# soasme/LTX-Video-GPUPoor

Hardware: AMD Instinct MI355X
Metric: denoise-steps/sec + VAE-decode frames/sec, LTX-Video 768x512x97f at 1/8 GPU (higher is better)
Workload: dtype bf16

## Files before the change

### include/ltxmi.h

```cpp
#ifndef LTXMI_H
#define LTXMI_H

#include <stddef.h>
#include <stdint.h>

#ifdef __cplusplus
extern "C" {
#endif

typedef enum ltxmi_status {
    LTXMI_OK = 0,
    LTXMI_ERR_INVALID_ARG = -1,
    LTXMI_ERR_UNSUPPORTED = -2,
    LTXMI_ERR_LAUNCH = -3
} ltxmi_status;

const char* ltxmi_version(void);
const char* ltxmi_last_error(void);
const char* ltxmi_arch(void);

typedef enum ltxmi_epilogue {
    LTXMI_EPI_NONE = 0,
    LTXMI_EPI_GELU_TANH = 1,
    LTXMI_EPI_SILU = 2,
// ... 37 lines not shown
                             const void* scale_table, const void* scale_temb,
                             const void* shift_table, const void* shift_temb,
                             int64_t temb_ld, int32_t rows_per_group, void* stream);

int ltxmi_norm_modulate_f32in_bf16(const float* x, int64_t ldx, void* y, int64_t ldy,
                                   int32_t rows, int32_t D, float eps, int32_t kind,
                                   const void* scale_table, const void* scale_temb,
                                   const void* shift_table, const void* shift_temb,
                                   int64_t temb_ld, int32_t rows_per_group, void* stream);

int ltxmi_gate_residual_f32(float* h, int64_t ldh, const void* y, int64_t ldy, int32_t rows, int32_t D,
                            const void* gate_table, const void* gate_temb, int64_t gate_ld,
                            int32_t rows_per_group, int32_t round_product,
                            void* h_bf16, int64_t ld_h_bf16, void* stream);

int ltxmi_rmsnorm_rope_bf16(void* x, int64_t ldx, int32_t rows, int32_t D,
                            const void* weight, float eps,
                            const void* cos_tab, const void* sin_tab, int64_t ld_tab,
                            int32_t rope_period, void* stream);
int ltxmi_rmsnorm_rope_rstd_bf16(void* x, int64_t ldx, int32_t rows, int32_t D, const void* weight, float eps,
                                 const void* cos_tab, const void* sin_tab, int64_t ld_tab, int32_t rope_period,
                                 const float* rowsumsq, int64_t rowsumsq_ld, int32_t rowsumsq_blocks,
                                 int32_t norm_dim, float norm_eps, float* rstd_out, void* stream);

typedef struct ltxmi_attn_args {
    const void* q; int64_t q_stride_b, q_stride_l;
    const void* k; int64_t k_stride_b, k_stride_l;
    const void* v; int64_t v_stride_b, v_stride_l;
    void*       o; int64_t o_stride_b, o_stride_l;
    const float* key_bias; int64_t bias_stride_b;
    int32_t B, H, Lq, Lk, head_dim;
    float   softmax_scale;
    const float* q_rowsumsq; int64_t q_rowsumsq_stride_b, q_rowsumsq_stride_l; int32_t q_rowsumsq_blocks;
    const void*  q_norm_weight; float q_norm_eps;
    const void*  rope_cos; const void* rope_sin; int64_t rope_stride_b, rope_stride_l;
    int32_t o_segment_len; int64_t o_stride_segment;
    const float* q_rstd; int64_t q_rstd_stride_b, q_rstd_stride_l;
    uint32_t* redo_counter; int32_t force_exact;
    float* lse; int64_t lse_stride_b, lse_stride_h;
} ltxmi_attn_args;

int ltxmi_attention_fwd_bf16(const ltxmi_attn_args* args, void* stream);
int ltxmi_attention_fuses_qnorm(int32_t B, int32_t H, int32_t Lq, int32_t Lk, int32_t head_dim, int32_t has_key_bias);
int ltxmi_attention_kernel_id(int32_t B, int32_t H, int32_t Lq, int32_t Lk, int32_t head_dim, int32_t has_key_bias,
                              int64_t k_stride_l, int64_t v_stride_l);

// ... 123 lines not shown
```

### ltx-video-gpupoor_amd/csrc/rowops.hip

```cpp
#include "common.h"

namespace ltxmi {

constexpr int ROWS_PER_WG = 4;

struct Chunk {
    float v[8];
};
__device__ __forceinline__ Chunk load_chunk(const uint16_t* p) {
    const u32x4 w = *(const u32x4*)p;
    Chunk c;
#pragma unroll
    for (int i = 0; i < 4; ++i) {
        c.v[2 * i] = bf_lo(w[i]);
        c.v[2 * i + 1] = bf_hi(w[i]);
    }
    return c;
}
__device__ __forceinline__ void store_chunk(uint16_t* p, const Chunk& c) {
    u32x4 w;
#pragma unroll
    for (int i = 0; i < 4; ++i) w[i] = pack_bf16(c.v[2 * i], c.v[2 * i + 1]);
    *(u32x4*)p = w;
}
// ... 88 lines not shown
    }
    s2 = wave_sum(s2);
    const float rstd = rsqrtf(s2 / D + eps);
    const int64_t trow = cs ? (int64_t)(row % rope_period) * ld_tab : 0;
#pragma unroll
    for (int j = 0; j < NCH; ++j) {
        const int ch = lane + 64 * j;
        if (ch < nchunk) {
            const Chunk wt = load_chunk(w + ch * 8);
            Chunk o;
#pragma unroll
            for (int e = 0; e < 8; ++e) o.v[e] = c[j].v[e] * rstd * wt.v[e];
            if (cs) {
                const Chunk co = load_chunk(cs + trow + ch * 8), si = load_chunk(sn + trow + ch * 8);
                Chunk r2;
#pragma unroll
                for (int e = 0; e < 8; e += 2) {
                    r2.v[e] = o.v[e] * co.v[e] - o.v[e + 1] * si.v[e];
                    r2.v[e + 1] = o.v[e + 1] * co.v[e + 1] + o.v[e] * si.v[e + 1];
                }
                o = r2;
            }
            store_chunk(xr + ch * 8, o);
        }
    }
}

template <int NCH>
__global__ __launch_bounds__(256) void pixelnorm_ada_silu_kernel(const uint16_t* __restrict__ x,
                                                                 uint16_t* __restrict__ y, int64_t rows, int C,
                                                                 int64_t rows_per_batch,
                                                                 const float* __restrict__ scale,
                                                                 const float* __restrict__ shift, int apply_silu,
                                                                 float eps) {
    const int lane = threadIdx.x & 63;
    const int64_t row = (int64_t)blockIdx.x * ROWS_PER_WG + (threadIdx.x >> 6);
    if (row >= rows) return;
    const int nchunk = C >> 3;
    const uint16_t* xr = x + row * C;
    Chunk c[NCH];
    float s2 = 0.f;
#pragma unroll
    for (int j = 0; j < NCH; ++j) {
        const int ch = lane + 64 * j;
        if (ch < nchunk) {
            c[j] = load_chunk(xr + ch * 8);
// ... 294 lines not shown
    return check_launch("ltxmi_rmsnorm_rope_bf16");
}

extern "C" int ltxmi_qkv_norm_rope_pack_bf16(const void* qkv, int64_t ld, int32_t B, int32_t Nl, int32_t D, int32_t P,
                                             const void* q_weight, const void* k_weight, float eps, const void* cos_tab,
                                             const void* sin_tab, int64_t ld_tab, int32_t rope_period, void* out,
                                             void* stream) {
    LTXMI_REQUIRE(qkv && q_weight && k_weight && out, LTXMI_ERR_INVALID_ARG, "ltxmi_qkv_norm_rope_pack_bf16: NULL argument");
    LTXMI_REQUIRE((cos_tab == nullptr) == (sin_tab == nullptr), LTXMI_ERR_INVALID_ARG,
                  "ltxmi_qkv_norm_rope_pack_bf16: cos and sin must both be given or both be NULL");
    LTXMI_REQUIRE(B > 0 && Nl > 0 && D > 0 && P > 0, LTXMI_ERR_INVALID_ARG, "ltxmi_qkv_norm_rope_pack_bf16: non-positive size");
    LTXMI_REQUIRE(D % (8 * P) == 0 && D <= 8192 && ld % 8 == 0 && ld >= 3 * D, LTXMI_ERR_UNSUPPORTED,
                  "ltxmi_qkv_norm_rope_pack_bf16: D=%d must be a multiple of 8 * P (P=%d) and <= 8192, ld >= 3 D", D, P);
    LTXMI_REQUIRE((int64_t)B * Nl < (1ll << 31) - 4, LTXMI_ERR_UNSUPPORTED, "ltxmi_qkv_norm_rope_pack_bf16: too many rows");
    if (cos_tab) LTXMI_REQUIRE(rope_period > 0 && ld_tab % 8 == 0 && ld_tab >= D, LTXMI_ERR_INVALID_ARG,
                               "ltxmi_qkv_norm_rope_pack_bf16: bad rope table geometry");
    const int rows = B * Nl, grid = (rows + ROWS_PER_WG - 1) / ROWS_PER_WG;
    hipStream_t s = (hipStream_t)stream;
    DISPATCH_NCH(D, hipLaunchKernelGGL((qkv_norm_rope_pack_kernel<NCH>), dim3(grid), dim3(256), 0, s, (const uint16_t*)qkv,
                                       ld, B, Nl, D, P, (const uint16_t*)q_weight, (const uint16_t*)k_weight, eps,
                                       (const uint16_t*)cos_tab, (const uint16_t*)sin_tab, ld_tab,
                                       rope_period > 0 ? rope_period : 1, (uint16_t*)out))
    return check_launch("ltxmi_qkv_norm_rope_pack_bf16");
}

extern "C" int ltxmi_pixelnorm_ada_silu_bf16(const void* x, void* y, int64_t rows, int32_t C,
                                             int64_t rows_per_batch, const float* scale, const float* shift,
                                             int32_t apply_silu, float eps, void* stream) {
    LTXMI_REQUIRE(x && y, LTXMI_ERR_INVALID_ARG, "ltxmi_pixelnorm_ada_silu_bf16: NULL argument");
    LTXMI_REQUIRE((scale == nullptr) == (shift == nullptr), LTXMI_ERR_INVALID_ARG,
                  "ltxmi_pixelnorm_ada_silu_bf16: scale and shift must both be given or both be NULL");
    LTXMI_REQUIRE(rows > 0 && C > 0 && rows_per_batch > 0, LTXMI_ERR_INVALID_ARG,
                  "ltxmi_pixelnorm_ada_silu_bf16: non-positive size");
    LTXMI_REQUIRE(C % 8 == 0 && C <= 8192, LTXMI_ERR_UNSUPPORTED,
                  "ltxmi_pixelnorm_ada_silu_bf16: C=%d must be a multiple of 8 and <= 8192", C);
    const int64_t grid = (rows + ROWS_PER_WG - 1) / ROWS_PER_WG;
    LTXMI_REQUIRE(grid < (1ll << 31), LTXMI_ERR_UNSUPPORTED, "ltxmi_pixelnorm_ada_silu_bf16: too many rows");
    hipStream_t s = (hipStream_t)stream;
    if ((C == 64 || C == 128 || C == 256) && ((((uintptr_t)scale | (uintptr_t)shift) & 15) == 0)) {
        const int rpw = 512 / C;
        int64_t g = (rows + ROWS_PER_WG * rpw - 1) / (ROWS_PER_WG * rpw);
        if (g > 256 * 16) g = 256 * 16;
#define CALLN(LPR_)                                                                                             \
    hipLaunchKernelGGL((pixelnorm_ada_silu_narrow_kernel<LPR_>), dim3((unsigned)g), dim3(256), 0, s,             \
                       (const uint16_t*)x, (uint16_t*)y, rows, rows_per_batch, scale, shift, apply_silu, eps)
        if (C == 64) CALLN(8);
// ... 26 lines not shown
```

### ltx-video-gpupoor_amd/ltxmi/_lib.py

```python
import ctypes
import os

import torch

_HERE = os.path.dirname(os.path.abspath(__file__))
LIB_PATH = os.environ.get("LTXMI_LIB") or os.path.join(_HERE, "libltxmi.so")

c_void_p, c_int, c_int64, c_float = ctypes.c_void_p, ctypes.c_int32, ctypes.c_int64, ctypes.c_float


class GemmArgs(ctypes.Structure):
    _fields_ = [("A", c_void_p), ("lda", c_int64), ("W", c_void_p), ("ldw", c_int64), ("bias", c_void_p),
                ("C", c_void_p), ("ldc", c_int64), ("M", c_int), ("N", c_int), ("K", c_int),
                ("epilogue", c_int), ("residual", c_void_p), ("ldr", c_int64), ("gate_table", c_void_p),
                ("gate_temb", c_void_p), ("gate_ld", c_int64), ("rows_per_group", c_int), ("algo", c_int),
                ("rowsumsq", c_void_p), ("rowsumsq_cols", c_int), ("rowsumsq_ld", c_int64),
                ("a_kblock", c_int), ("a_kblock_stride", c_int64)]


class GemmPair(ctypes.Structure):
    _fields_ = [("A2", c_void_p), ("lda2", c_int64), ("W2", c_void_p), ("ldw2", c_int64), ("K2", c_int), ("group_cols", c_int)]


class AttnArgs(ctypes.Structure):
    _fields_ = [("q", c_void_p), ("q_stride_b", c_int64), ("q_stride_l", c_int64),
                ("k", c_void_p), ("k_stride_b", c_int64), ("k_stride_l", c_int64),
                ("v", c_void_p), ("v_stride_b", c_int64), ("v_stride_l", c_int64),
                ("o", c_void_p), ("o_stride_b", c_int64), ("o_stride_l", c_int64),
                ("key_bias", c_void_p), ("bias_stride_b", c_int64),
                ("B", c_int), ("H", c_int), ("Lq", c_int), ("Lk", c_int), ("head_dim", c_int),
                ("softmax_scale", c_float),
                ("q_rowsumsq", c_void_p), ("q_rowsumsq_stride_b", c_int64), ("q_rowsumsq_stride_l", c_int64),
                ("q_rowsumsq_blocks", c_int), ("q_norm_weight", c_void_p), ("q_norm_eps", c_float),
                ("rope_cos", c_void_p), ("rope_sin", c_void_p), ("rope_stride_b", c_int64), ("rope_stride_l", c_int64),
                ("o_segment_len", c_int), ("o_stride_segment", c_int64),
                ("q_rstd", c_void_p), ("q_rstd_stride_b", c_int64), ("q_rstd_stride_l", c_int64),
                ("redo_counter", c_void_p), ("force_exact", c_int),
                ("lse", c_void_p), ("lse_stride_b", c_int64), ("lse_stride_h", c_int64)]


ATTN_MERGE_MAX = 8


class AttnMergeArgs(ctypes.Structure):
    _fields_ = [("n", c_int),
                ("o_part", c_void_p * ATTN_MERGE_MAX), ("o_part_stride_b", c_int64 * ATTN_MERGE_MAX),
                ("o_part_stride_l", c_int64 * ATTN_MERGE_MAX),
                ("lse_part", c_void_p * ATTN_MERGE_MAX), ("lse_part_stride_b", c_int64 * ATTN_MERGE_MAX),
                ("lse_part_stride_h", c_int64 * ATTN_MERGE_MAX),
                ("o", c_void_p), ("o_stride_b", c_int64), ("o_stride_l", c_int64),
                ("lse", c_void_p), ("lse_stride_b", c_int64), ("lse_stride_h", c_int64),
                ("B", c_int), ("H", c_int), ("Lq", c_int), ("head_dim", c_int)]


class Conv3dArgs(ctypes.Structure):
    _fields_ = [("x", c_void_p), ("w", c_void_p), ("bias", c_void_p), ("y", c_void_p),
                ("B", c_int), ("T", c_int), ("H", c_int), ("W", c_int), ("Cin", c_int), ("Cout", c_int),
                ("causal", c_int), ("pad_replicate", c_int), ("d2s", c_int), ("residual", c_void_p),
                ("res_channels", c_int), ("add", c_void_p),
                ("stride_t", c_int), ("stride_hw", c_int), ("tpad", c_int), ("out_T", c_int),
                ("kernel_t", c_int), ("time_pad_zeros", c_int), ("algo", c_int),
# ... 3 lines not shown

class Conv3dRouteInfo(ctypes.Structure):
    _fields_ = [("route", c_int), ("epilogue", c_int), ("ksplit", c_int), ("swap_hw", c_int), ("finalize_blocks", c_int)]


SIGNATURES = {
    "ltxmi_version": (ctypes.c_char_p, []),
    "ltxmi_last_error": (ctypes.c_char_p, []),
    "ltxmi_arch": (ctypes.c_char_p, []),
    "ltxmi_gemm_bf16": (c_int, [ctypes.POINTER(GemmArgs), c_void_p]),
    "ltxmi_gemm_kernel_id": (c_int, [ctypes.POINTER(GemmArgs)]),
    "ltxmi_gemm_pair2_bf16": (c_int, [ctypes.POINTER(GemmArgs), ctypes.POINTER(GemmPair), c_void_p]),
    "ltxmi_gemm_pair2_kernel_id": (c_int, [ctypes.POINTER(GemmArgs), ctypes.POINTER(GemmPair)]),
    "ltxmi_norm_modulate_bf16": (c_int, [c_void_p, c_int64, c_void_p, c_int64, c_int, c_int, c_float, c_int,
                                         c_void_p, c_void_p, c_void_p, c_void_p, c_int64, c_int, c_void_p]),
    "ltxmi_norm_modulate_f32in_bf16": (c_int, [c_void_p, c_int64, c_void_p, c_int64, c_int, c_int, c_float, c_int,
                                               c_void_p, c_void_p, c_void_p, c_void_p, c_int64, c_int, c_void_p]),
    "ltxmi_gate_residual_f32": (c_int, [c_void_p, c_int64, c_void_p, c_int64, c_int, c_int, c_void_p, c_void_p, c_int64,
                                        c_int, c_int, c_void_p, c_int64, c_void_p]),
    "ltxmi_rmsnorm_rope_bf16": (c_int, [c_void_p, c_int64, c_int, c_int, c_void_p, c_float, c_void_p, c_void_p,
                                        c_int64, c_int, c_void_p]),
    "ltxmi_rmsnorm_rope_rstd_bf16": (c_int, [c_void_p, c_int64, c_int, c_int, c_void_p, c_float, c_void_p, c_void_p,
                                             c_int64, c_int, c_void_p, c_int64, c_int, c_int, c_float, c_void_p, c_void_p]),
    "ltxmi_rowsumsq_rstd_f32": (c_int, [c_void_p, c_int64, c_int, c_int, c_int, c_float, c_void_p, c_void_p]),
    "ltxmi_qkv_norm_rope_pack_bf16": (c_int, [c_void_p, c_int64, c_int, c_int, c_int, c_int, c_void_p, c_void_p, c_float,
                                              c_void_p, c_void_p, c_int64, c_int, c_void_p, c_void_p]),
    "ltxmi_attention_fwd_bf16": (c_int, [ctypes.POINTER(AttnArgs), c_void_p]),
    "ltxmi_attention_merge_bf16": (c_int, [ctypes.POINTER(AttnMergeArgs), c_void_p]),
    "ltxmi_attention_fuses_qnorm": (c_int, [c_int, c_int, c_int, c_int, c_int, c_int]),
    "ltxmi_attention_kernel_id": (c_int, [c_int, c_int, c_int, c_int, c_int, c_int, c_int64, c_int64]),
    "ltxmi_silu_bf16": (c_int, [c_void_p, c_void_p, c_int64, c_void_p]),
    "ltxmi_timestep_embedding_bf16": (c_int, [c_void_p, c_void_p, c_int, c_int, c_void_p]),
    "ltxmi_stg_blend_bf16": (c_int, [c_void_p, c_int64, c_void_p, c_int64, c_void_p, c_int, c_int, c_int, c_void_p]),
    "ltxmi_stg_blend_grouped_bf16": (c_int, [c_void_p, c_void_p, c_int64, c_int64, c_int64, c_void_p, c_int, c_int, c_int, c_int,
                                             c_void_p]),
    "ltxmi_conv3d_ndhwc_bf16": (c_int, [ctypes.POINTER(Conv3dArgs), c_void_p]),
    "ltxmi_conv3d_fuses_post_norm": (c_int, [ctypes.POINTER(Conv3dArgs)]),
    "ltxmi_conv3d_workspace_bytes": (c_int64, [ctypes.POINTER(Conv3dArgs)]),
    "ltxmi_conv3d_route": (c_int, [ctypes.POINTER(Conv3dArgs), ctypes.POINTER(Conv3dRouteInfo)]),
    "ltxmi_pixelnorm_ada_silu_bf16": (c_int, [c_void_p, c_void_p, c_int64, c_int, c_int64, c_void_p, c_void_p,
                                              c_int, c_float, c_void_p]),
    "ltxmi_add_bf16": (c_int, [c_void_p, c_void_p, c_void_p, c_int64, c_void_p]),
    "ltxmi_layernorm_affine_bf16": (c_int, [c_void_p, c_void_p, c_int64, c_int, c_void_p, c_void_p, c_float,
                                            c_void_p]),
    "ltxmi_ncdhw_to_ndhwc_bf16": (c_int, [c_void_p, c_void_p, c_int, c_int, c_int, c_int, c_int, c_void_p,
                                          c_void_p, c_void_p]),
# ... 52 lines not shown
```

### ltx-video-gpupoor_amd/ltxmi/attention.py

```python
from enum import Enum, auto
from typing import Optional

import torch
from torch import nn

from . import lora, ops
from .attention_seam import pay_attention

BF16 = torch.bfloat16


FUSE_CROSS_ATTENTION_Q = True


class SkipLayerStrategy(Enum):
    AttentionSkip = auto()
    AttentionValues = auto()
    Residual = auto()
    TransformerBlock = auto()


def reshape_hidden_states(hidden_states, latent_frames):
    return hidden_states.reshape(hidden_states.shape[0], latent_frames, -1, hidden_states.shape[-1])

# ... 165 lines not shown
        else:
            wqkv, bqkv = attn.packed_qkv()
        if not isinstance(attn.q_norm, RMSNorm):
            raise NotImplementedError("ltxmi.AttnProcessor2_0: qk_norm=None is not on this path")

        q_fused = None
        if not is_cross:
            fuse_q = ops.attention_fuses_qnorm(B, H, N, N, dh) and D % 64 == 0 and attention_mask is None
            ss = torch.empty((B * N, D // 64), dtype=torch.float32, device=x2.device) if fuse_q else None
            qkv = ops.gemm(x2, wqkv, bqkv, rowsumsq=ss, rowsumsq_cols=D if fuse_q else 0,
                           **lora.pair(attn, "qkv", x2))
            q2, k2, v2 = qkv[:, :D], qkv[:, D:2 * D], qkv[:, 2 * D:]
            cos = sin = None
            period = 0
            if attn.use_rope:
                cos, sin = freqs_cis
                if cos.shape[0] not in (1, B):
                    raise ValueError("freqs_cis batch must be 1 or the batch size")
                cos2, sin2 = cos.reshape(-1, D), sin.reshape(-1, D)
                period = cos2.shape[0]
                cos, sin = cos2, sin2
            if fuse_q:
                rstd = torch.empty((B * N,), dtype=torch.float32, device=x2.device)
                ops.rmsnorm_rope_(k2, attn.k_norm.weight, attn.k_norm.eps, cos, sin, period,
                                  rstd_of=(ss, D, attn.q_norm.eps, rstd))
                q_fused = ((rstd, attn.q_norm.weight, attn.q_norm.eps), (cos, sin, period) if cos is not None else None)
            else:
                ops.rmsnorm_rope_(q2, attn.q_norm.weight, attn.q_norm.eps, cos, sin, period)
                ops.rmsnorm_rope_(k2, attn.k_norm.weight, attn.k_norm.eps, cos, sin, period)
            Lk = N
            q4 = qkv.view(B, N, 3, H, dh)[:, :, 0]
            k4 = qkv.view(B, N, 3, H, dh)[:, :, 1]
            v4 = qkv.view(B, N, 3, H, dh)[:, :, 2]
            v3 = qkv.view(B, N, 3 * D)[:, :, 2 * D:]
        else:
            Bk, Lk, _ = encoder_hidden_states.shape
            fuse_q = FUSE_CROSS_ATTENTION_Q and D % 64 == 0 and bool(ops.attention_fuses_qnorm(B, H, N, Lk, dh, attention_mask is not None))
            ss = torch.empty((B * N, D // 64), dtype=torch.float32, device=x2.device) if fuse_q else None
            q2 = ops.gemm(x2, attn.to_q.weight, attn.to_q.bias, rowsumsq=ss, rowsumsq_cols=D if fuse_q else 0,
                          **lora.pair(attn, "q", x2))
            ehs = encoder_hidden_states
            key = (ehs.data_ptr(), tuple(ehs.shape), ops.tensor_version(ehs), wkv.data_ptr(), ops.tensor_version(wkv),
                   attn.k_norm.weight.data_ptr(), ops.tensor_version(attn.k_norm.weight), lora.epoch(attn))
            cache = attn.__dict__.setdefault("_text_kv_cache", {})
            hit = cache.get(key) if ops.STEP_INVARIANT_CACHING else None
            if hit is None:
                ready = attn.__dict__.get("_text_kv_ready")
                if ready is not None:
# ... 205 lines not shown
```

### ltx-video-gpupoor_amd/ltxmi/ops.py

```python
import ctypes
import math

import torch

from . import _lib
from ._lib import lib, check

BF16 = torch.bfloat16

EPI_NONE, EPI_GELU_TANH, EPI_SILU, EPI_GATE_RESIDUAL = 0, 1, 2, 3
NORM_RMS, NORM_LAYER = 0, 1


def _stream():
    return ctypes.c_void_p(torch.cuda.current_stream().cuda_stream)


_watch = None
_events = {}


def watch_launches(keys):
    global _watch
    _watch = set(keys) if keys else None
# ... 200 lines not shown
    _chk_f32(h, "gate_residual_f32_")
    _chk_bf16(y, gate_table, gate_temb, h_bf16)
    h2, rows, ldh = _rows(h)
    y2, yrows, ldy = _rows(y)
    D = h2.shape[1]
    if yrows != rows or y2.shape[1] != D:
        raise ValueError("ltxmi.gate_residual_f32_: y must have h's rows and channels")
    if (gate_table is None) != (gate_temb is None):
        raise ValueError("ltxmi.gate_residual_f32_: gate_table and gate_temb go together")
    gate_ld = 0
    if gate_temb is not None:
        gate_ld = gate_temb.stride(0) if gate_temb.dim() == 2 else 0
    b2, ldb = None, 0
    if h_bf16 is not None:
        b2, brows, ldb = _rows(h_bf16)
        if brows != rows or b2.shape[1] != D:
            raise ValueError("ltxmi.gate_residual_f32_: h_bf16 must have h's rows and channels")
    check(lib.ltxmi_gate_residual_f32(_ptr(h2), ldh, _ptr(y2), ldy, rows, D, _ptr(gate_table), _ptr(gate_temb), gate_ld,
                                      rows_per_group, int(round_product), _ptr(b2), ldb, _stream()),
          "ltxmi_gate_residual_f32")
    return h


def rmsnorm_rope_(x, weight, eps, cos=None, sin=None, rope_period=0, rstd_of=None):
    _chk_bf16(x, weight, cos, sin)
    x2, rows, ldx = _rows(x)
    D = x2.shape[1]
    ld_tab = 0
    if cos is not None:
        if cos.dim() != 2 or cos.shape != sin.shape or cos.stride(0) != sin.stride(0):
            raise ValueError("ltxmi.rmsnorm_rope_: cos/sin must be matching 2-D tables")
        ld_tab = cos.stride(0)
        rope_period = rope_period or cos.shape[0]
    if rstd_of is not None:
        ss, norm_dim, norm_eps, out = rstd_of
        if ss.dtype != torch.float32 or out.dtype != torch.float32 or ss.dim() != 2 or ss.shape[0] != rows or \
                ss.stride(1) != 1 or out.shape != (rows,) or not out.is_contiguous():
            raise ValueError("ltxmi.rmsnorm_rope_: rstd_of needs fp32 sums [rows, blocks] and a contiguous fp32 out [rows]")
        check(lib.ltxmi_rmsnorm_rope_rstd_bf16(_ptr(x2), ldx, rows, D, _ptr(weight), eps, _ptr(cos), _ptr(sin), ld_tab,
                                               rope_period, _ptr(ss), ss.stride(0), ss.shape[1], norm_dim, norm_eps,
                                               _ptr(out), _stream()), "ltxmi_rmsnorm_rope_rstd_bf16")
        return x
    check(lib.ltxmi_rmsnorm_rope_bf16(_ptr(x2), ldx, rows, D, _ptr(weight), eps, _ptr(cos), _ptr(sin), ld_tab,
                                      rope_period, _stream()), "ltxmi_rmsnorm_rope_bf16")
    return x


def rowsumsq_rstd(ss, norm_dim, eps, out=None):
    if ss.dtype != torch.float32 or ss.dim() != 2 or ss.stride(1) != 1 or not ss.is_cuda:
        raise ValueError("ltxmi.rowsumsq_rstd: expected CUDA fp32 sums [rows, blocks]")
    rows = ss.shape[0]
    out = torch.empty((rows,), dtype=torch.float32, device=ss.device) if out is None else out
    check(lib.ltxmi_rowsumsq_rstd_f32(_ptr(ss), ss.stride(0), ss.shape[1], rows, norm_dim, eps, _ptr(out), _stream()),
          "ltxmi_rowsumsq_rstd_f32")
    return out


def attention_fuses_qnorm(B, H, Lq, Lk, dh, has_key_bias=False):
    return bool(lib.ltxmi_attention_fuses_qnorm(B, H, Lq, Lk, dh, int(has_key_bias)))


# ... 543 lines not shown
```

### ltx-video-gpupoor_amd/ltxmi/transformer3d.py

```python
import contextlib
import math
from dataclasses import dataclass
from typing import Any, Dict, List, Optional

import torch
from torch import nn

from . import lora, ops
from .attention import BasicTransformerBlock, SkipLayerStrategy

BF16 = torch.bfloat16


@dataclass
class Transformer3DModelOutput:
    sample: torch.Tensor


class _TimestepEmbedder(nn.Module):
    def __init__(self, in_channels, dim):
        super().__init__()
        self.linear_1 = nn.Linear(in_channels, dim)
        self.linear_2 = nn.Linear(dim, dim)

# ... 196 lines not shown
            sin_freq = torch.cat([torch.zeros_like(cos_freq[:, :, : dim % 6]), sin_freq], dim=-1)
        return cos_freq.to(self.dtype).contiguous(), sin_freq.to(self.dtype).contiguous()

    def _stacked_text_kv(self, ehs):
        blocks = [b for b in self.transformer_blocks if getattr(b, "attn2", None) is not None]
        if not blocks or ehs.dim() != 3 or not ehs.is_contiguous():
            return
        if any(lora.has_slot(b.attn2, "kv") for b in blocks):
            return
        packs = [b.attn2.packed_kv() for b in blocks]
        if any(bk is None for _, bk in packs) or len({tuple(w.shape) for w, _ in packs}) != 1:
            return
        key = tuple((w.data_ptr(), ops.tensor_version(w), bk.data_ptr(), ops.tensor_version(bk)) for w, bk in packs)
        st = self.__dict__.get("_stacked_kv_weights")
        if st is None or st[0] != key:
            with torch.no_grad():
                st = (key, torch.cat([w for w, _ in packs], 0).contiguous(), torch.cat([bk for _, bk in packs], 0).contiguous(),
                      packs)
            self.__dict__["_stacked_kv_weights"] = st
        _, w_all, b_all, _ = st
        Bk, Lk, _ = ehs.shape
        two_d = packs[0][0].shape[0]
        kv_all = ops.gemm(ehs.reshape(Bk * Lk, -1), w_all, b_all)
        for i, b in enumerate(blocks):
            kv = kv_all[:, i * two_d:(i + 1) * two_d]
            ops.rmsnorm_rope_(kv[:, :two_d // 2], b.attn2.k_norm.weight, b.attn2.k_norm.eps)
            b.attn2.__dict__["_text_kv_ready"] = (ehs, ops.tensor_version(ehs), kv, lora.epoch(b.attn2))

    def _run_blocks_microbatched(self, hidden_states, slices, freqs_cis, attention_mask, encoder_hidden_states,
                                 encoder_attention_mask, temb, cross_attention_kwargs, class_labels, layer_mask,
                                 skip_layer_strategy, ltxv_model):
        B = hidden_states.shape[0]
        on_gpu = hidden_states.is_cuda
        streams = None
        for block in self.transformer_blocks:
            block.prepare_shared_state()
        if on_gpu:
            main = torch.cuda.current_stream()
            key = (hidden_states.device, len(slices))
            pool = self.__dict__.setdefault("_mb_streams", {})
            streams = pool.get(key)
            if streams is None:
                streams = pool[key] = [torch.cuda.Stream(device=hidden_states.device) for _ in slices]
            for st in streams:
                st.wait_stream(main)

        def rows(t, sl):
            return t if (t is None or t.shape[0] != B) else t[sl]

# ... 8 lines not shown
                          cross_attention_kwargs=cross_attention_kwargs, class_labels=class_labels,
                          skip_layer_mask=layer_mask(block_idx, sl), skip_layer_strategy=skip_layer_strategy)
            if ltxv_model is not None and ltxv_model._interrupt:
                interrupted = True
                break
        if on_gpu:
            for st in streams:
                main.wait_stream(st)
        return interrupted

    def forward(self, hidden_states: torch.Tensor, freqs_cis: list,
                encoder_hidden_states: Optional[torch.Tensor] = None, timestep: Optional[torch.Tensor] = None,
                class_labels: Optional[torch.LongTensor] = None, cross_attention_kwargs: Dict[str, Any] = None,
                attention_mask: Optional[torch.Tensor] = None, encoder_attention_mask: Optional[torch.Tensor] = None,
                skip_layer_mask: Optional[torch.Tensor] = None,
                skip_layer_strategy: Optional[SkipLayerStrategy] = None, latent_shape=None, joint_pass=True,
                ltxv_model=None, mixed=False, return_dict: bool = True, stg_alias_blocks: int = 0,
                stg_alias_rows: int = 1, _microbatches=None):
        if self.dtype != BF16:
            raise TypeError("ltxmi.Transformer3DModel runs in bfloat16 only: call .to(torch.bfloat16)")
        if attention_mask is not None:
            raise NotImplementedError("a self-attention mask is not on this path")
        dtype = self.dtype
        hidden_states = hidden_states.to(dtype)
        B, N, _ = hidden_states.shape
        D = self.inner_dim

        if encoder_attention_mask is not None and encoder_attention_mask.ndim == 2:
            encoder_attention_mask = ((1 - encoder_attention_mask.to(dtype)) * -10000.0).unsqueeze(1)

        hidden_states = ops.gemm(hidden_states.reshape(B * N, -1), self.patchify_proj.weight,
                                 self.patchify_proj.bias).view(B, N, D)

        timestep = timestep.to(torch.float32)
        if self.timestep_scale_multiplier:
            timestep = self.timestep_scale_multiplier * timestep
        if timestep.shape[-1] > 1:
            timestep = timestep.reshape(timestep.shape[0], -1, latent_shape[-2] * latent_shape[-1])[:, :, 0]
        temb, embedded_timestep = self.adaln_single(timestep.flatten())
        temb = temb.view(B, -1, 6 * D)
        embedded_timestep = embedded_timestep.view(B, -1, D)
        if mixed:
            hidden_states = hidden_states.float()

        if self.caption_projection is not None:
            ehs = encoder_hidden_states
# ... 100 lines not shown
```

Before: 16.65.

## Add grouped text-K RMSNorm and optional packed cos/sin RoPE kernel

Replaces the per-block loop of text cross-attention K RMSNorm launches with one grouped kernel that normalizes every block's K slice in a single launch, using a 2-D grid with per-group weights. It also adds an opt-in path, off by default through an environment variable, that packs cos and sin into one interleaved bf16 table. A shared-row RMSNorm+RoPE kernel then keeps the RoPE row in registers across rows with the same period and prefetches the next row. The grouped path cuts launch overhead at the cost of a new kernel, and the packed path adds a pack kernel plus a device-side fallback flag.

```diff
diff --git a/include/ltxmi.h b/include/ltxmi.h
--- a/include/ltxmi.h
+++ b/include/ltxmi.h
@@ -83,6 +83,21 @@
                                  const void* cos_tab, const void* sin_tab, int64_t ld_tab, int32_t rope_period,
                                  const float* rowsumsq, int64_t rowsumsq_ld, int32_t rowsumsq_blocks,
                                  int32_t norm_dim, float norm_eps, float* rstd_out, void* stream);
+
+int ltxmi_rope_pack_bf16(const void* cos_tab, const void* sin_tab, int64_t ld_tab, int32_t rows, int32_t D,
+                         void* packed, int64_t ld_packed, int32_t* bad, void* stream);
+
+#define LTXMI_RMSNORM_GROUPS_MAX 32
+typedef struct ltxmi_rmsnorm_rope_args {
+    void* x; int64_t ldx;
+    int32_t rows, D;
+    const void* weight; float eps;
+    const void* cos_tab; const void* sin_tab; int64_t ld_tab; int32_t rope_period;
+    const float* rowsumsq; int64_t rowsumsq_ld; int32_t rowsumsq_blocks, norm_dim; float norm_eps; float* rstd_out;
+    const void* rope_packed; int64_t ld_packed; const int32_t* rope_packed_bad;
+    int32_t groups; int64_t group_stride; const void* const* group_weights;
+} ltxmi_rmsnorm_rope_args;
+int ltxmi_rmsnorm_rope_args_bf16(const ltxmi_rmsnorm_rope_args* args, void* stream);
 
 typedef struct ltxmi_attn_args {
     const void* q; int64_t q_stride_b, q_stride_l;
diff --git a/ltx-video-gpupoor_amd/csrc/rowops.hip b/ltx-video-gpupoor_amd/csrc/rowops.hip
--- a/ltx-video-gpupoor_amd/csrc/rowops.hip
+++ b/ltx-video-gpupoor_amd/csrc/rowops.hip
@@ -134,6 +134,175 @@
                 o = r2;
             }
             store_chunk(xr + ch * 8, o);
+        }
+    }
+}
+
+__global__ __launch_bounds__(256) void rope_pack_kernel(const uint16_t* __restrict__ cs, const uint16_t* __restrict__ sn,
+                                                        int64_t ld_tab, int rows, int nchunk, uint16_t* __restrict__ out,
+                                                        int64_t ld_out, int* __restrict__ bad) {
+    const int64_t i = (int64_t)blockIdx.x * 256 + threadIdx.x;
+    if (i >= (int64_t)rows * nchunk) return;
+    const int64_t r = i / nchunk;
+    const int ch = (int)(i - r * nchunk);
+    const u32x4 c = *(const u32x4*)(cs + r * ld_tab + ch * 8), s = *(const u32x4*)(sn + r * ld_tab + ch * 8);
+    u32x4 o;
+    bool differ = false;
+#pragma unroll
+    for (int k = 0; k < 4; ++k) {
+        differ |= (c[k] >> 16) != (c[k] & 0xffffu) || (s[k] >> 16) != (s[k] & 0xffffu);
+        o[k] = (c[k] & 0xffffu) | (s[k] << 16);
+    }
+    *(u32x4*)(out + r * ld_out + ch * 8) = o;
+    if (differ) *bad = 1;
+}
+
+__device__ __forceinline__ float pinned(float v) {
+    asm volatile("" : "+v"(v));
+    return v;
+}
+template <bool FIRST>
+__device__ __forceinline__ float chunk_sumsq(const Chunk& c) {
+    float lo = c.v[6] * c.v[6], hi = c.v[7] * c.v[7];
+    lo = __builtin_fmaf(c.v[2], c.v[2], pinned(lo));
+    hi = __builtin_fmaf(c.v[3], c.v[3], pinned(hi));
+    lo = __builtin_fmaf(c.v[4], c.v[4], lo);
+    hi = __builtin_fmaf(c.v[5], c.v[5], hi);
+    lo = __builtin_fmaf(c.v[FIRST ? 1 : 0], c.v[FIRST ? 1 : 0], lo);
+    hi = __builtin_fmaf(c.v[FIRST ? 0 : 1], c.v[FIRST ? 0 : 1], hi);
+    return pinned(pinned(lo) + pinned(hi));
+}
+__device__ __forceinline__ Chunk chunk_scale(const Chunk& c, float rstd, const Chunk& wt) {
+    Chunk o;
+#pragma unroll
+    for (int e = 0; e < 8; ++e) o.v[e] = pinned(pinned(c.v[e] * rstd) * wt.v[e]);
+    return o;
+}
+__device__ __forceinline__ Chunk chunk_rotate(const Chunk& o, const Chunk& co, const Chunk& si) {
+    Chunk r;
+#pragma unroll
+    for (int e = 0; e < 8; e += 2) {
+        r.v[e] = __builtin_fmaf(o.v[e], co.v[e], -pinned(o.v[e + 1] * si.v[e]));
+        r.v[e + 1] = __builtin_fmaf(o.v[e], si.v[e + 1], pinned(o.v[e + 1] * co.v[e + 1]));
+    }
+    return r;
+}
+
+template <int NCH>
+__global__ __launch_bounds__(256) void rmsnorm_rope_shared_kernel(uint16_t* __restrict__ x, int64_t ldx, int rows, int D,
+                                                                  const uint16_t* __restrict__ w, float eps,
+                                                                  const uint16_t* __restrict__ pk, int64_t ld_pk,
+                                                                  const int* __restrict__ pk_bad,
+                                                                  const uint16_t* __restrict__ cs,
+                                                                  const uint16_t* __restrict__ sn, int64_t ld_tab, int period,
+                                                                  const float* __restrict__ side_ss, int64_t side_ld, int side_n,
+                                                                  float side_inv_d, float side_eps,
+                                                                  float* __restrict__ side_rstd) {
+    const int lane = threadIdx.x & 63;
+    const int64_t t64 = (int64_t)blockIdx.x * ROWS_PER_WG + (threadIdx.x >> 6);
+    if (t64 >= period || t64 >= rows) return;
+    const int t = (int)t64;
+    const bool use_pk = pk_bad == nullptr || *pk_bad == 0;
+    const int nchunk = D >> 3;
+    u32x4 tab[NCH], nxt[NCH];
+#pragma unroll
+    for (int j = 0; j < NCH; ++j) {
+        const int ch = lane + 64 * j;
+        tab[j] = u32x4{0u, 0u, 0u, 0u};
+        nxt[j] = u32x4{0u, 0u, 0u, 0u};
+        if (ch < nchunk) {
+            if (use_pk) tab[j] = *(const u32x4*)(pk + (int64_t)t * ld_pk + ch * 8);
+            nxt[j] = *(const u32x4*)(x + (int64_t)t * ldx + ch * 8);
+        }
+    }
+    const int64_t trow = (int64_t)t * ld_tab;
+    for (int row = t;; row += period) {
+        const bool more = rows - row > period;
+        uint16_t* xr = x + (int64_t)row * ldx;
+        Chunk c[NCH];
+#pragma unroll
+        for (int j = 0; j < NCH; ++j) {
+#pragma unroll
+            for (int i = 0; i < 4; ++i) {
+                c[j].v[2 * i] = bf_lo(nxt[j][i]);
+                c[j].v[2 * i + 1] = bf_hi(nxt[j][i]);
+            }
+        }
+        if (more) {
+            const uint16_t* xn = xr + (int64_t)period * ldx;
+#pragma unroll
+            for (int j = 0; j < NCH; ++j) {
+                const int ch = lane + 64 * j;
+                if (ch < nchunk) nxt[j] = *(const u32x4*)(xn + ch * 8);
+            }
+        }
+        if (side_ss) {
+            float s = 0.f;
+            for (int j = lane; j < side_n; j += 64) s += side_ss[(int64_t)row * side_ld + j];
+            s = wave_sum(s);
+            if (lane == 0) side_rstd[row] = rsqrtf(s * side_inv_d + side_eps);
+        }
+        float s2 = 0.f;
+#pragma unroll
+        for (int j = 0; j < NCH; ++j) {
+            if (lane + 64 * j < nchunk) s2 = pinned(s2 + (j == 0 ? chunk_sumsq<true>(c[j]) : chunk_sumsq<false>(c[j])));
+        }
+        s2 = wave_sum(s2);
+        const float rstd = rsqrtf(s2 / D + eps);
+#pragma unroll
+        for (int j = 0; j < NCH; ++j) {
+            const int ch = lane + 64 * j;
+            if (ch < nchunk) {
+                const Chunk wt = load_chunk(w + ch * 8);
+                const Chunk o = chunk_scale(c[j], rstd, wt);
+                Chunk co, si;
+                if (use_pk) {
+#pragma unroll
+                    for (int i = 0; i < 4; ++i) {
+                        co.v[2 * i] = co.v[2 * i + 1] = bf_lo(tab[j][i]);
+                        si.v[2 * i] = si.v[2 * i + 1] = bf_hi(tab[j][i]);
+                    }
+                } else {
+                    co = load_chunk(cs + trow + ch * 8);
+                    si = load_chunk(sn + trow + ch * 8);
+                }
+                store_chunk(xr + ch * 8, chunk_rotate(o, co, si));
+            }
+        }
+        if (!more) break;
+    }
+}
+
+struct GroupWeights {
+    const uint16_t* p[LTXMI_RMSNORM_GROUPS_MAX];
+};
+template <int NCH>
+__global__ __launch_bounds__(256) void rmsnorm_grouped_kernel(uint16_t* __restrict__ x, int64_t ldx, int rows, int D,
+                                                              int64_t group_stride, GroupWeights w, float eps) {
+    const int lane = threadIdx.x & 63;
+    const int64_t row = (int64_t)blockIdx.x * ROWS_PER_WG + (threadIdx.x >> 6);
+    if (row >= rows) return;
+    const uint16_t* wg = w.p[blockIdx.y];
+    const int nchunk = D >> 3;
+    uint16_t* xr = x + (int64_t)row * ldx + (int64_t)blockIdx.y * group_stride;
+    Chunk c[NCH];
+    float s2 = 0.f;
+#pragma unroll
+    for (int j = 0; j < NCH; ++j) {
+        const int ch = lane + 64 * j;
+        if (ch < nchunk) {
+            c[j] = load_chunk(xr + ch * 8);
+            s2 = pinned(s2 + (j == 0 ? chunk_sumsq<true>(c[j]) : chunk_sumsq<false>(c[j])));
+        }
+    }
+    s2 = wave_sum(s2);
+    const float rstd = rsqrtf(s2 / D + eps);
+#pragma unroll
+    for (int j = 0; j < NCH; ++j) {
+        const int ch = lane + 64 * j;
+        if (ch < nchunk) {
+            const Chunk wt = load_chunk(wg + ch * 8);
+            store_chunk(xr + ch * 8, chunk_scale(c[j], rstd, wt));
         }
     }
 }
@@ -474,6 +643,98 @@
                                        (const uint16_t*)cos_tab, (const uint16_t*)sin_tab, ld_tab,
                                        rope_period > 0 ? rope_period : 1, (uint16_t*)out))
     return check_launch("ltxmi_qkv_norm_rope_pack_bf16");
+}
+
+extern "C" int ltxmi_rope_pack_bf16(const void* cos_tab, const void* sin_tab, int64_t ld_tab, int32_t rows, int32_t D,
+                                    void* packed, int64_t ld_packed, int32_t* bad, void* stream) {
+    LTXMI_REQUIRE(cos_tab && sin_tab && packed && bad, LTXMI_ERR_INVALID_ARG, "ltxmi_rope_pack_bf16: NULL argument");
+    LTXMI_REQUIRE(rows > 0 && D > 0, LTXMI_ERR_INVALID_ARG, "ltxmi_rope_pack_bf16: non-positive size rows=%d D=%d", rows, D);
+    LTXMI_REQUIRE(D % 8 == 0 && ld_tab % 8 == 0 && ld_packed % 8 == 0 && ld_tab >= D && ld_packed >= D &&
+                      ((((uintptr_t)cos_tab) | ((uintptr_t)sin_tab) | ((uintptr_t)packed)) & 15) == 0 && (((uintptr_t)bad) & 3) == 0,
+                  LTXMI_ERR_UNSUPPORTED,
+                  "ltxmi_rope_pack_bf16: D=%d and the row strides must be multiples of 8 and >= D, the tables 16-byte aligned", D);
+    const int64_t chunks = (int64_t)rows * (D >> 3);
+    LTXMI_REQUIRE((chunks + 255) / 256 < (1ll << 31), LTXMI_ERR_UNSUPPORTED, "ltxmi_rope_pack_bf16: table too large");
+    hipLaunchKernelGGL(rope_pack_kernel, dim3((unsigned)((chunks + 255) / 256)), dim3(256), 0, (hipStream_t)stream,
+                       (const uint16_t*)cos_tab, (const uint16_t*)sin_tab, ld_tab, rows, D >> 3, (uint16_t*)packed, ld_packed,
+                       (int*)bad);
+    return check_launch("ltxmi_rope_pack_bf16");
+}
+
+extern "C" int ltxmi_rmsnorm_rope_args_bf16(const ltxmi_rmsnorm_rope_args* a, void* stream) {
+    LTXMI_REQUIRE(a, LTXMI_ERR_INVALID_ARG, "ltxmi_rmsnorm_rope_args_bf16: NULL args");
+    hipStream_t s = (hipStream_t)stream;
+    if (a->groups != 0) {
+        LTXMI_REQUIRE(a->x && a->group_weights, LTXMI_ERR_INVALID_ARG, "ltxmi_rmsnorm_rope_args_bf16: NULL x / group_weights");
+        LTXMI_REQUIRE(a->groups > 0 && a->groups <= LTXMI_RMSNORM_GROUPS_MAX, LTXMI_ERR_INVALID_ARG,
+                      "ltxmi_rmsnorm_rope_args_bf16: groups=%d outside 1 .. %d", a->groups, LTXMI_RMSNORM_GROUPS_MAX);
+        LTXMI_REQUIRE(!a->cos_tab && !a->sin_tab && !a->rope_packed && !a->rowsumsq && !a->rstd_out, LTXMI_ERR_INVALID_ARG,
+                      "ltxmi_rmsnorm_rope_args_bf16: the grouped form takes no RoPE table and no rowsumsq / rstd_out");
+        LTXMI_REQUIRE(a->rows > 0 && a->D > 0, LTXMI_ERR_INVALID_ARG, "ltxmi_rmsnorm_rope_args_bf16: non-positive size");
+        LTXMI_REQUIRE(a->D % 8 == 0 && a->D <= 2048 && a->ldx % 8 == 0 && a->group_stride % 8 == 0 && a->group_stride >= a->D &&
+                          a->ldx >= (int64_t)(a->groups - 1) * a->group_stride + a->D && (((uintptr_t)a->x) & 15) == 0,
+                      LTXMI_ERR_UNSUPPORTED,
+                      "ltxmi_rmsnorm_rope_args_bf16: grouped form needs D=%d %% 8 == 0 and <= 2048, D <= group_stride, all groups "
+                      "inside a row, strides multiples of 8, x 16-byte aligned", a->D);
+        GroupWeights gw;
+        for (int g = 0; g < LTXMI_RMSNORM_GROUPS_MAX; ++g) gw.p[g] = nullptr;
+        for (int g = 0; g < a->groups; ++g) {
+            LTXMI_REQUIRE(a->group_weights[g], LTXMI_ERR_INVALID_ARG, "ltxmi_rmsnorm_rope_args_bf16: group_weights[%d] is NULL", g);
+            LTXMI_REQUIRE((((uintptr_t)a->group_weights[g]) & 15) == 0, LTXMI_ERR_UNSUPPORTED,
+                          "ltxmi_rmsnorm_rope_args_bf16: group_weights[%d] is not 16-byte aligned", g);
+            gw.p[g] = (const uint16_t*)a->group_weights[g];
+        }
+        const unsigned grid = (unsigned)(((int64_t)a->rows + ROWS_PER_WG - 1) / ROWS_PER_WG);
+        if (a->D <= 512)
+            hipLaunchKernelGGL((rmsnorm_grouped_kernel<1>), dim3(grid, a->groups), dim3(256), 0, s, (uint16_t*)a->x, a->ldx,
+                               a->rows, a->D, a->group_stride, gw, a->eps);
+        else
+            hipLaunchKernelGGL((rmsnorm_grouped_kernel<4>), dim3(grid, a->groups), dim3(256), 0, s, (uint16_t*)a->x, a->ldx,
+                               a->rows, a->D, a->group_stride, gw, a->eps);
+        return check_launch("ltxmi_rmsnorm_rope_args_bf16");
+    }
+    if (a->rowsumsq || a->rstd_out) {
+        LTXMI_REQUIRE(a->rowsumsq && a->rstd_out, LTXMI_ERR_INVALID_ARG,
+                      "ltxmi_rmsnorm_rope_args_bf16: rowsumsq and rstd_out must both be given or both be NULL");
+        LTXMI_REQUIRE(a->rowsumsq_blocks > 0 && a->norm_dim > 0 && a->rowsumsq_ld >= a->rowsumsq_blocks &&
+                          ((((uintptr_t)a->rowsumsq) | ((uintptr_t)a->rstd_out)) & 3) == 0,
+                      LTXMI_ERR_INVALID_ARG, "ltxmi_rmsnorm_rope_args_bf16: bad rowsumsq geometry (blocks %d, ld %lld, dim %d)",
+                      a->rowsumsq_blocks, (long long)a->rowsumsq_ld, a->norm_dim);
+    }
+    const int side_d = a->rowsumsq ? a->norm_dim : 1;
+    if (!a->rope_packed)
+        return rmsnorm_rope_launch(a->x, a->ldx, a->rows, a->D, a->weight, a->eps, a->cos_tab, a->sin_tab, a->ld_tab,
+                                   a->rope_period, a->rowsumsq, a->rowsumsq_ld, a->rowsumsq_blocks, side_d, a->norm_eps,
+                                   a->rstd_out, stream);
+    LTXMI_REQUIRE(a->x && a->weight, LTXMI_ERR_INVALID_ARG, "ltxmi_rmsnorm_rope_args_bf16: NULL argument");
+    LTXMI_REQUIRE((a->cos_tab == nullptr) == (a->sin_tab == nullptr), LTXMI_ERR_INVALID_ARG,
+                  "ltxmi_rmsnorm_rope_args_bf16: cos and sin must both be given or both be NULL");
+    LTXMI_REQUIRE(a->rope_packed_bad == nullptr || a->cos_tab != nullptr, LTXMI_ERR_INVALID_ARG,
+                  "ltxmi_rmsnorm_rope_args_bf16: rope_packed_bad needs the unpacked cos / sin tables to fall back on");
+    LTXMI_REQUIRE(a->rows > 0 && a->D > 0 && a->rope_period > 0, LTXMI_ERR_INVALID_ARG,
+                  "ltxmi_rmsnorm_rope_args_bf16: non-positive size or rope_period");
+    LTXMI_REQUIRE(a->D % 8 == 0 && a->D <= 2048 && a->ldx % 8 == 0 && a->ldx >= a->D && (!a->rowsumsq || a->rowsumsq_blocks <= 64),
+                  LTXMI_ERR_UNSUPPORTED,
+                  "ltxmi_rmsnorm_rope_args_bf16: with rope_packed D=%d must be a multiple of 8 and <= 2048, ldx >= D, and "
+                  "rowsumsq_blocks <= 64", a->D);
+    LTXMI_REQUIRE(a->ld_packed % 8 == 0 && a->ld_packed >= a->D && (((uintptr_t)a->rope_packed) & 15) == 0 &&
+                      (((uintptr_t)a->rope_packed_bad) & 3) == 0 && ((((uintptr_t)a->x) | ((uintptr_t)a->weight)) & 15) == 0,
+                  LTXMI_ERR_INVALID_ARG, "ltxmi_rmsnorm_rope_args_bf16: bad packed rope table geometry");
+    if (a->cos_tab)
+        LTXMI_REQUIRE(a->ld_tab % 8 == 0 && a->ld_tab >= a->D && ((((uintptr_t)a->cos_tab) | ((uintptr_t)a->sin_tab)) & 15) == 0,
+                      LTXMI_ERR_INVALID_ARG, "ltxmi_rmsnorm_rope_args_bf16: bad rope table geometry");
+    const int waves = a->rope_period < a->rows ? a->rope_period : a->rows;
+    const unsigned grid = (unsigned)(((int64_t)waves + ROWS_PER_WG - 1) / ROWS_PER_WG);
+#define CALLS(N_)                                                                                                        \
+    hipLaunchKernelGGL((rmsnorm_rope_shared_kernel<N_>), dim3(grid), dim3(256), 0, s, (uint16_t*)a->x, a->ldx, a->rows,   \
+                       a->D, (const uint16_t*)a->weight, a->eps, (const uint16_t*)a->rope_packed, a->ld_packed,           \
+                       (const int*)a->rope_packed_bad, (const uint16_t*)a->cos_tab, (const uint16_t*)a->sin_tab,          \
+                       a->ld_tab, a->rope_period, a->rowsumsq, a->rowsumsq_ld, a->rowsumsq_blocks, 1.0f / (float)side_d,  \
+                       a->norm_eps, a->rstd_out)
+    if (a->D <= 512) CALLS(1);
+    else CALLS(4);
+#undef CALLS
+    return check_launch("ltxmi_rmsnorm_rope_args_bf16");
 }
 
 extern "C" int ltxmi_pixelnorm_ada_silu_bf16(const void* x, void* y, int64_t rows, int32_t C,
diff --git a/ltx-video-gpupoor_amd/ltxmi/_lib.py b/ltx-video-gpupoor_amd/ltxmi/_lib.py
--- a/ltx-video-gpupoor_amd/ltxmi/_lib.py
+++ b/ltx-video-gpupoor_amd/ltxmi/_lib.py
@@ -37,6 +37,18 @@
                 ("q_rstd", c_void_p), ("q_rstd_stride_b", c_int64), ("q_rstd_stride_l", c_int64),
                 ("redo_counter", c_void_p), ("force_exact", c_int),
                 ("lse", c_void_p), ("lse_stride_b", c_int64), ("lse_stride_h", c_int64)]
+
+
+RMSNORM_GROUPS_MAX = 32
+
+
+class RmsnormRopeArgs(ctypes.Structure):
+    _fields_ = [("x", c_void_p), ("ldx", c_int64), ("rows", c_int), ("D", c_int), ("weight", c_void_p), ("eps", c_float),
+                ("cos_tab", c_void_p), ("sin_tab", c_void_p), ("ld_tab", c_int64), ("rope_period", c_int),
+                ("rowsumsq", c_void_p), ("rowsumsq_ld", c_int64), ("rowsumsq_blocks", c_int), ("norm_dim", c_int),
+                ("norm_eps", c_float), ("rstd_out", c_void_p),
+                ("rope_packed", c_void_p), ("ld_packed", c_int64), ("rope_packed_bad", c_void_p),
+                ("groups", c_int), ("group_stride", c_int64), ("group_weights", ctypes.POINTER(c_void_p))]
 
 
 ATTN_MERGE_MAX = 8
@@ -86,6 +98,8 @@
                                         c_int64, c_int, c_void_p]),
     "ltxmi_rmsnorm_rope_rstd_bf16": (c_int, [c_void_p, c_int64, c_int, c_int, c_void_p, c_float, c_void_p, c_void_p,
                                              c_int64, c_int, c_void_p, c_int64, c_int, c_int, c_float, c_void_p, c_void_p]),
+    "ltxmi_rope_pack_bf16": (c_int, [c_void_p, c_void_p, c_int64, c_int, c_int, c_void_p, c_int64, c_void_p, c_void_p]),
+    "ltxmi_rmsnorm_rope_args_bf16": (c_int, [ctypes.POINTER(RmsnormRopeArgs), c_void_p]),
     "ltxmi_rowsumsq_rstd_f32": (c_int, [c_void_p, c_int64, c_int, c_int, c_int, c_float, c_void_p, c_void_p]),
     "ltxmi_qkv_norm_rope_pack_bf16": (c_int, [c_void_p, c_int64, c_int, c_int, c_int, c_int, c_void_p, c_void_p, c_float,
                                               c_void_p, c_void_p, c_int64, c_int, c_void_p, c_void_p]),
diff --git a/ltx-video-gpupoor_amd/ltxmi/attention.py b/ltx-video-gpupoor_amd/ltxmi/attention.py
--- a/ltx-video-gpupoor_amd/ltxmi/attention.py
+++ b/ltx-video-gpupoor_amd/ltxmi/attention.py
@@ -211,8 +211,11 @@
                 cos, sin = cos2, sin2
             if fuse_q:
                 rstd = torch.empty((B * N,), dtype=torch.float32, device=x2.device)
+                pack = {}
+                if cos is not None and ops.ROPE_PACKED and cos.is_cuda and D <= ops.ROPE_PACKED_MAX_D:
+                    pack = dict(packed=ops.rope_pack(cos, sin))
                 ops.rmsnorm_rope_(k2, attn.k_norm.weight, attn.k_norm.eps, cos, sin, period,
-                                  rstd_of=(ss, D, attn.q_norm.eps, rstd))
+                                  rstd_of=(ss, D, attn.q_norm.eps, rstd), **pack)
                 q_fused = ((rstd, attn.q_norm.weight, attn.q_norm.eps), (cos, sin, period) if cos is not None else None)
             else:
                 ops.rmsnorm_rope_(q2, attn.q_norm.weight, attn.q_norm.eps, cos, sin, period)
diff --git a/ltx-video-gpupoor_amd/ltxmi/ops.py b/ltx-video-gpupoor_amd/ltxmi/ops.py
--- a/ltx-video-gpupoor_amd/ltxmi/ops.py
+++ b/ltx-video-gpupoor_amd/ltxmi/ops.py
@@ -1,5 +1,6 @@
 import ctypes
 import math
+import os
 
 import torch
 
@@ -246,7 +247,65 @@
     return h
 
 
-def rmsnorm_rope_(x, weight, eps, cos=None, sin=None, rope_period=0, rstd_of=None):
+ROPE_PACKED = os.environ.get("LTXMI_ROPE_PACKED", "0") == "1"
+TEXT_K_GROUPED = True
+ROPE_PACKED_MAX_D = 2048
+_rope_packs = {}
+_forward_epoch = 0
+
+
+class PackedRope:
+    __slots__ = ("table", "bad", "cos", "sin")
+
+    def __init__(self, table, bad, cos, sin):
+        self.table, self.bad, self.cos, self.sin = table, bad, cos, sin
+
+    def is_valid(self):
+        return int(self.bad.item()) == 0
+
+
+def begin_forward():
+    global _forward_epoch
+    _forward_epoch += 1
+
+
+def rope_pack(cos, sin):
+    _chk_bf16(cos, sin)
+    if cos.dim() != 2 or cos.shape != sin.shape or cos.stride(0) != sin.stride(0) or cos.stride(1) != 1 or sin.stride(1) != 1:
+        raise ValueError("ltxmi.rope_pack: cos/sin must be matching 2-D tables with contiguous rows")
+    key = (cos.data_ptr(), sin.data_ptr(), tensor_version(cos), tensor_version(sin), tuple(cos.shape), cos.stride(0), cos.device,
+           None if STEP_INVARIANT_CACHING else _forward_epoch)
+    hit = _rope_packs.get(key)
+    if hit is not None:
+        return hit
+    rows, D = cos.shape
+    table = torch.empty((rows, D), dtype=BF16, device=cos.device)
+    bad = torch.zeros((1,), dtype=torch.int32, device=cos.device)
+    check(lib.ltxmi_rope_pack_bf16(_ptr(cos), _ptr(sin), cos.stride(0), rows, D, _ptr(table), D, _ptr(bad), _stream()),
+          "ltxmi_rope_pack_bf16")
+    if len(_rope_packs) >= 4:
+        _rope_packs.clear()
+    hit = _rope_packs[key] = PackedRope(table, bad, cos, sin)
+    return hit
+
+
+def rmsnorm_grouped_(x, weights, eps, D, group_stride):
+    _chk_bf16(x, *weights)
+    x2, rows, ldx = _rows(x)
+    G = len(weights)
+    if G < 1 or x2.shape[1] < (G - 1) * group_stride + D or any(w.shape != (D,) or not w.is_contiguous() for w in weights):
+        raise ValueError("ltxmi.rmsnorm_grouped_: x must hold every group's D columns, weights must be contiguous [D]")
+    for g0 in range(0, G, _lib.RMSNORM_GROUPS_MAX):
+        ws = weights[g0:g0 + _lib.RMSNORM_GROUPS_MAX]
+        a = _lib.RmsnormRopeArgs()
+        a.x, a.ldx, a.rows, a.D, a.eps = x2.data_ptr() + g0 * group_stride * x2.element_size(), ldx, rows, D, eps
+        a.groups, a.group_stride = len(ws), group_stride
+        a.group_weights = (ctypes.c_void_p * len(ws))(*[w.data_ptr() for w in ws])
+        check(lib.ltxmi_rmsnorm_rope_args_bf16(ctypes.byref(a), _stream()), "ltxmi_rmsnorm_rope_args_bf16")
+    return x
+
+
+def rmsnorm_rope_(x, weight, eps, cos=None, sin=None, rope_period=0, rstd_of=None, packed=None):
     _chk_bf16(x, weight, cos, sin)
     x2, rows, ldx = _rows(x)
     D = x2.shape[1]
@@ -261,6 +320,20 @@
         if ss.dtype != torch.float32 or out.dtype != torch.float32 or ss.dim() != 2 or ss.shape[0] != rows or \
                 ss.stride(1) != 1 or out.shape != (rows,) or not out.is_contiguous():
             raise ValueError("ltxmi.rmsnorm_rope_: rstd_of needs fp32 sums [rows, blocks] and a contiguous fp32 out [rows]")
+    if packed is not None:
+        if cos is None or packed.cos.data_ptr() != cos.data_ptr() or packed.sin.data_ptr() != sin.data_ptr() or \
+                tuple(packed.table.shape) != tuple(cos.shape) or packed.cos.stride(0) != cos.stride(0):
+            raise ValueError("ltxmi.rmsnorm_rope_: packed must be rope_pack(cos, sin) of the tables given")
+        a = _lib.RmsnormRopeArgs()
+        a.x, a.ldx, a.rows, a.D, a.weight, a.eps = x2.data_ptr(), ldx, rows, D, weight.data_ptr(), eps
+        a.cos_tab, a.sin_tab, a.ld_tab, a.rope_period = cos.data_ptr(), sin.data_ptr(), ld_tab, rope_period
+        a.rope_packed, a.ld_packed, a.rope_packed_bad = packed.table.data_ptr(), packed.table.stride(0), packed.bad.data_ptr()
+        if rstd_of is not None:
+            a.rowsumsq, a.rowsumsq_ld, a.rowsumsq_blocks = ss.data_ptr(), ss.stride(0), ss.shape[1]
+            a.norm_dim, a.norm_eps, a.rstd_out = norm_dim, norm_eps, out.data_ptr()
+        check(lib.ltxmi_rmsnorm_rope_args_bf16(ctypes.byref(a), _stream()), "ltxmi_rmsnorm_rope_args_bf16")
+        return x
+    if rstd_of is not None:
         check(lib.ltxmi_rmsnorm_rope_rstd_bf16(_ptr(x2), ldx, rows, D, _ptr(weight), eps, _ptr(cos), _ptr(sin), ld_tab,
                                                rope_period, _ptr(ss), ss.stride(0), ss.shape[1], norm_dim, norm_eps,
                                                _ptr(out), _stream()), "ltxmi_rmsnorm_rope_rstd_bf16")
diff --git a/ltx-video-gpupoor_amd/ltxmi/transformer3d.py b/ltx-video-gpupoor_amd/ltxmi/transformer3d.py
--- a/ltx-video-gpupoor_amd/ltxmi/transformer3d.py
+++ b/ltx-video-gpupoor_amd/ltxmi/transformer3d.py
@@ -242,9 +242,14 @@
         Bk, Lk, _ = ehs.shape
         two_d = packs[0][0].shape[0]
         kv_all = ops.gemm(ehs.reshape(Bk * Lk, -1), w_all, b_all)
+        grouped = ops.TEXT_K_GROUPED and kv_all.is_cuda and two_d // 2 <= ops.ROPE_PACKED_MAX_D and len({b.attn2.k_norm.eps for b in blocks}) == 1
+        if grouped:
+            ops.rmsnorm_grouped_(kv_all, [b.attn2.k_norm.weight for b in blocks], blocks[0].attn2.k_norm.eps,
+                                 two_d // 2, two_d)
         for i, b in enumerate(blocks):
             kv = kv_all[:, i * two_d:(i + 1) * two_d]
-            ops.rmsnorm_rope_(kv[:, :two_d // 2], b.attn2.k_norm.weight, b.attn2.k_norm.eps)
+            if not grouped:
+                ops.rmsnorm_rope_(kv[:, :two_d // 2], b.attn2.k_norm.weight, b.attn2.k_norm.eps)
             b.attn2.__dict__["_text_kv_ready"] = (ehs, ops.tensor_version(ehs), kv, lora.epoch(b.attn2))
 
     def _run_blocks_microbatched(self, hidden_states, slices, freqs_cis, attention_mask, encoder_hidden_states,
@@ -299,6 +304,7 @@
         if attention_mask is not None:
             raise NotImplementedError("a self-attention mask is not on this path")
         dtype = self.dtype
+        ops.begin_forward()
         hidden_states = hidden_states.to(dtype)
         B, N, _ = hidden_states.shape
         D = self.inner_dim
```

Result: no change. 16.63 (-0.1%).
